# NVIDIA/OpenSeq2Seq

Hardware: AMD Instinct MI355X
Metric: audio-frames/sec/node Jasper10x5 bf16 (train step, objects = input feature frames) (higher is better)
Workload: dtype bf16; 1 GPU; Jasper 10x5 DR (jasper10x5_LibriSpeech_nvgrad_masks) full train step: log-mel front end from int16 PCM resident in HBM+fwd+bwd+NovoGrad/LARC/Backoff, B=32/GPU, durations U[2,16.7]s padded to the batch max, F=64, V=29; global_batch=32, parallelism=dp1, skipped_steps=0

## Files before the change

### openseq2seq_amd/csrc/conv1d_wgrad.hip

```cpp
#include <stdlib.h>

#include <cstdlib>
#include "os2s_common.hpp"
#include "os2s_split_reduce.hpp"
#include <mutex>

namespace os2s {

struct WgradArgs {
  const bf16_t* x;
  const bf16_t* dy;
  float* dw;
  const int32_t* in_len;
  int B, Tin, Tout, Cin, Cout, K, stride, dil, padL;
  int NCO, NCI, NTP, NSPLIT, steps_per_split, use_atomic;
  float* part;
  int xrows, xrows_pad;
  int xbuf_bytes, steptab_bytes;
  long long x_ld;
  int accumulate;
  float* ws_slabs;
  int* ws_cnt;
  int ws_nslabs, ncu, force_split;
  int xcd_order;
  int NG;
  const bf16_t* gx[8];
  const bf16_t* gdy[8];
  float* gdw[8];
  unsigned long long* dbg;
  int dbg_mode;
};

__device__ __forceinline__ int wgrad_xcd_rank(int b, int n) {
  const int q = n >> 3, r = n & 7, x = b & 7;
  return (x < r ? x * (q + 1) : r * (q + 1) + (x - r) * q) + (b >> 3);
}

__device__ __forceinline__ void dma16w(const void* gsrc, char* lds_wave_base) {
  __builtin_amdgcn_global_load_lds(
      (const __attribute__((address_space(1))) void*)gsrc,
      (__attribute__((address_space(3))) void*)lds_wave_base, 16, 0, 0);
}

__device__ __forceinline__ bf16x4 lds_tr(const char* p) {
  return __builtin_amdgcn_ds_read_tr16_b64_v4bf16(
      (__attribute__((address_space(3))) bf16x4*)p);
}

template <int TAPS, int COT>
__device__ __forceinline__ void wgrad_lockstep_unit(const WgradArgs& p, const int unit, const int tp, char* smem) {
  constexpr int BT = 64;
  constexpr int NW = COT / 32, NTHR = NW * 64, NSUB = COT / 128;
  const int tid = threadIdx.x, lane = tid & 63;
  const int wid = __builtin_amdgcn_readfirstlane(tid >> 6);
  const int wm = wid >> 1, wn = wid & 1;
  const int ysub = wm >> 1, wmi = wm & 1;
  const int split = unit / (p.NCO * p.NCI);
  const int rem = unit - split * (p.NCO * p.NCI);
  const int co0 = (rem / p.NCI) * COT, ci0 = (rem % p.NCI) * 128;
  const int k0 = tp * TAPS;
  const int ntaps = min(TAPS, p.K - k0);

  const int ybuf_bytes = NSUB * BT * 256;
  const int xbuf_bytes = p.xrows_pad * 256;
  char* const ybuf0 = smem;
  char* const xbuf0 = smem + 2 * ybuf_bytes;
  const char* const zero = reinterpret_cast<const char*>(g_zero_page);

  const int tchunks = (p.Tout + BT - 1) / BT;
  auto nlive = [&](int b) -> int {
    if (!p.in_len) return tchunks;
    const int l = min(max(p.in_len[b], 0), p.Tin);
    if (l <= 0) return 0;
    return min(tchunks, (l + p.padL + BT * p.stride - 1) / (BT * p.stride));
  };
  int total_live = 0;
  for (int b = 0; b < p.B; ++b) total_live += nlive(b);
  const int sps = (total_live + p.NSPLIT - 1) / p.NSPLIT;
  const int s_begin = split * sps;
  const int s_end = min(total_live, s_begin + sps);
  const int nsteps = max(0, s_end - s_begin);
  int cur_b = 0, cur_c = 0;
  {
    int acc_steps = 0;
    while (cur_b < p.B && acc_steps + nlive(cur_b) <= s_begin) { acc_steps += nlive(cur_b); ++cur_b; }
    cur_c = s_begin - acc_steps;
  }

  auto stage = [&](int step, int buf) {
    const int b = min(cur_b, p.B - 1);
    const int t0 = cur_c * BT;
    ++cur_c;
    if (cur_c >= nlive(b)) {
      cur_c = 0;
      ++cur_b;
      while (cur_b < p.B && nlive(cur_b) == 0) ++cur_b;
    }
    int len_b = p.Tin;
    if (p.in_len) {
      int l = p.in_len[b];
      len_b = l < 0 ? 0 : (l < p.Tin ? l : p.Tin);
    }
    char* yd = ybuf0 + buf * ybuf_bytes;
    const bf16_t* dyb = p.dy + (long long)b * p.Tout * p.Cout;
#pragma unroll
    for (int it = 0; it < (NSUB * 16) / NW; ++it) {
      const int base = (it * NW + wid) * 64;
// ... 142 lines not shown
  const bf16_t* x;
  const bf16_t* dy;
  float* dw;
  long long x_ld;
  int Cin, Cout, NCI, unit_begin;
};
struct WgradGroupTable {
  int ngroups, total_units;
  WgradGroup g[kMaxWgradGroups];
};

__global__ __launch_bounds__(256, 2) void conv1d_wgrad_grouped_kernel(WgradArgs p, WgradGroupTable gt) {
  extern __shared__ __attribute__((aligned(16))) char smem[];
  const int bid = blockIdx.x;
  if (bid >= gt.total_units) return;
  int gi = 0;
#pragma unroll
  for (int i = 1; i < kMaxWgradGroups; ++i)
    if (i < gt.ngroups && bid >= gt.g[i].unit_begin) gi = i;
  WgradGroup g = gt.g[0];
#pragma unroll
  for (int i = 1; i < kMaxWgradGroups; ++i)
    if (i == gi) g = gt.g[i];
  p.x = g.x; p.dy = g.dy; p.dw = g.dw; p.x_ld = g.x_ld;
  p.Cin = g.Cin; p.Cout = g.Cout;
  p.NCO = (g.Cout + 127) / 128; p.NCI = g.NCI;
  wgrad_lockstep_unit<1, 128>(p, bid - g.unit_begin, 0, smem);
}

template <int OFF>
__device__ __forceinline__ bf16x4 lds_tr_asm(unsigned addr) {
  bf16x4 v;
  asm volatile("ds_read_b64_tr_b16 %0, %1 offset:%2" : "=v"(v) : "v"(addr), "n"(OFF) : "memory");
  return v;
}
template <int KK>
__device__ __forceinline__ bf16x8 lds_frag(unsigned addr) {
  const bf16x4 lo = lds_tr_asm<KK * 4096>(addr);
  const bf16x4 hi = lds_tr_asm<KK * 4096 + 1024>(addr);
  return __builtin_shufflevector(lo, hi, 0, 1, 2, 3, 4, 5, 6, 7);
}

__device__ __forceinline__ void wpp_barrier() {
  __builtin_amdgcn_sched_barrier(0);
  __builtin_amdgcn_s_barrier();
  __builtin_amdgcn_sched_barrier(0);
}

constexpr int kWppTaps = 4;
struct WppStaged {
  unsigned ylo, yhi, ynr, xlo, xhi, xnr;
  int xro;
};

template <bool DBG>
__global__ __launch_bounds__(512, 2) void conv1d_wgrad_pp_kernel(WgradArgs p) {
  constexpr int BT = 64, COT = 128, CIT = 128;
  constexpr int YBUF = BT * 256;
  extern __shared__ __attribute__((aligned(16))) char smem[];
  const int tid = threadIdx.x, lane = tid & 63;
  const int wid = __builtin_amdgcn_readfirstlane(tid >> 6);
  const int grp = wid >> 2, wq = wid & 3;
  const int wm = wq >> 1, wn = wq & 1;

  const int tchunks = (p.Tout + BT - 1) / BT;
  int nl = 0, len_l = 0;
  if (lane < p.B) {
    len_l = p.Tin;
    if (p.in_len) {
      const int l = p.in_len[lane];
      len_l = l < 0 ? 0 : (l < p.Tin ? l : p.Tin);
    }
    nl = len_l > 0 ? (len_l + p.padL + BT - 1) / BT : 0;
    nl = nl < tchunks ? nl : tchunks;
  }
  int scan = nl;
#pragma unroll
  for (int o = 1; o < 64; o <<= 1) {
    const int t = __shfl_up(scan, o, 64);
    if (lane >= o) scan += t;
  }
  const int total_live = __builtin_amdgcn_readlane(scan, 63);

  const int U = p.NG * p.NCO * p.NCI * p.NTP, G = p.ncu;
  const int q = U / G, r = U - q * G;
  int f = 1;
  {
    int fmax = total_live / 8;
    fmax = fmax > 16 ? 16 : fmax;
    if (p.force_split > 0 && p.ws_slabs) {
      f = p.force_split < fmax ? p.force_split : (fmax > 1 ? fmax : 1);
      while (f > 1 && r * f > p.ws_nslabs) --f;
      if (r == 0) f = 1;
    } else if (r > 0 && p.ws_slabs) {
      f = split_factor(r, G, 1.1f * total_live, fmax, p.ws_nslabs);
    }
  }
  const int nfull = f > 1 ? U - r : U;
  const int nwork = nfull + (f > 1 ? r * f : 0);
  if ((int)blockIdx.x >= nwork) return;
  const int bid = p.xcd_order ? wgrad_xcd_rank(blockIdx.x, nwork) : (int)blockIdx.x;
  int rank = bid, piece = 0, npiece = 1;
  if (bid >= nfull) {
    const int i = bid - nfull;
    rank = nfull + i / f;
    piece = i - (i / f) * f;
    npiece = f;
  }
  const int tp = rank % p.NTP;
  int rem = rank / p.NTP;
  if (p.NG > 1) {
    const int per = p.NCO * p.NCI;
    const int g = __builtin_amdgcn_readfirstlane(rem / per);
    rem -= g * per;
    const bf16_t* sx = p.gx[0]; const bf16_t* sdy = p.gdy[0]; float* sdw = p.gdw[0];
#pragma unroll
    for (int i = 1; i < 8; ++i)
      if (i == g) { sx = p.gx[i]; sdy = p.gdy[i]; sdw = p.gdw[i]; }
    p.x = sx; p.dy = sdy; p.dw = sdw;
  }
  const int co0 = (rem / p.NCI) * COT, ci0 = (rem % p.NCI) * CIT;
  const int k0 = tp * kWppTaps;
  const int sps = (total_live + npiece - 1) / npiece;
  const int s_begin = __builtin_amdgcn_readfirstlane(min(piece * sps, total_live));
  const int s_end = __builtin_amdgcn_readfirstlane(min(total_live, s_begin + sps));
  const int nsteps = s_end - s_begin;

  const int xbuf_bytes = p.xbuf_bytes;
  char* const ybuf0 = smem;
  char* const xbuf0 = smem + 2 * YBUF;
  int* const steptab = reinterpret_cast<int*>(xbuf0 + 3 * xbuf_bytes);

  {
    const int excl = scan - nl;
    for (int c = 0; c < tchunks; ++c) {
      const int idx = excl + c - s_begin;
      if (lane < p.B && c < nl && idx >= 0 && idx < nsteps && wid == 0)
        steptab[idx] = lane | (c << 8) | (len_l << 16);
    }
  }

  int yv[2];
#pragma unroll
  for (int it = 0; it < 2; ++it) {
    const int qq = (it * 8 + wid) * 64 + lane;
    const int row = qq >> 4, ps = qq & 15;
    const int u = (ps >> 1) ^ ((row & 3) << 1);
    const int ch = co0 + ((u << 1) | (ps & 1)) * 8;
    yv[it] = ch < p.Cout ? (row * p.Cout + ch) * 2 : (int)0x80000000;
  }
  int xv[3];
#pragma unroll
  for (int n = 0; n < 3; ++n) {
    const int qq = (n * 8 + wid) * 64 + lane;
    const int row = qq >> 4, ps = qq & 15;
    const int u = (ps >> 1) ^ ((row & 3) << 1);
    const int ch = ci0 + ((u << 1) | (ps & 1)) * 8;
    xv[n] = (ch < p.Cin && row < p.xrows) ? (row * (int)p.x_ld + ch) * 2 : (int)0x80000000;
  }
  const bool x3 = 16 + wid < ((p.xrows * 16 + 63) >> 6);
  const unsigned long long dy_base = (unsigned long long)p.dy, x_base = (unsigned long long)p.x;
  const int ycol_bytes = __builtin_amdgcn_readfirstlane(p.Cout * 2);
  const int xcol_bytes = __builtin_amdgcn_readfirstlane((int)p.x_ld * 2);
  const unsigned long long xsample_bytes = (unsigned long long)p.Tin * (unsigned long long)p.x_ld * 2ull;
  auto prep = [&](int ent) __attribute__((always_inline)) -> WppStaged {
    const int b = ent & 0xff, t0 = ((ent >> 8) & 0xff) * BT, len_b = (int)((unsigned)ent >> 16);
    WppStaged st;
    const unsigned long long yb = dy_base + (unsigned long long)(unsigned)(b * p.Tout + t0) * (unsigned)ycol_bytes;
    st.ylo = (unsigned)yb; st.yhi = (unsigned)(yb >> 32);
    st.ynr = (unsigned)((p.Tout - t0) * ycol_bytes);
    const unsigned long long xb = x_base + (unsigned long long)(unsigned)b * xsample_bytes;
    st.xlo = (unsigned)xb; st.xhi = (unsigned)(xb >> 32);
    st.xnr = (unsigned)(len_b * xcol_bytes);
    st.xro = (t0 + k0 * p.dil - p.padL) * xcol_bytes;
#if defined(__HIP_DEVICE_COMPILE__)
    asm volatile("" : "+s"(st.ylo), "+s"(st.yhi), "+s"(st.ynr), "+s"(st.xlo), "+s"(st.xhi), "+s"(st.xnr), "+s"(st.xro));
#endif
    return st;
  };
  auto issue = [&](const WppStaged& st, int ybuf_idx, int xbuf_idx) __attribute__((always_inline)) {
    const __amdgpu_buffer_rsrc_t yrs = __builtin_amdgcn_make_buffer_rsrc(
        (void*)(((unsigned long long)st.yhi << 32) | st.ylo), 0, (int)st.ynr, 0x00020000);
    const __amdgpu_buffer_rsrc_t xrs = __builtin_amdgcn_make_buffer_rsrc(
        (void*)(((unsigned long long)st.xhi << 32) | st.xlo), 0, (int)st.xnr, 0x00020000);
    char* const yd = ybuf0 + ybuf_idx * YBUF;
    if (!(DBG && (p.dbg_mode & 1)))
#pragma unroll
    for (int it = 0; it < 2; ++it)
      __builtin_amdgcn_raw_ptr_buffer_load_lds(
          yrs, (__attribute__((address_space(3))) void*)(yd + (it * 8 + wid) * 1024), 16, yv[it], 0, 0, 0);
    char* const xd = xbuf0 + xbuf_idx * xbuf_bytes;
    if (!(DBG && (p.dbg_mode & 2))) {
#pragma unroll
      for (int n = 0; n < 2; ++n)
        __builtin_amdgcn_raw_ptr_buffer_load_lds(
            xrs, (__attribute__((address_space(3))) void*)(xd + (n * 8 + wid) * 1024), 16,
            xv[n] + st.xro, 0, 0, 0);
      if (x3)
        __builtin_amdgcn_raw_ptr_buffer_load_lds(
            xrs, (__attribute__((address_space(3))) void*)(xd + (16 + wid) * 1024), 16, xv[2] + st.xro, 0, 0, 0);
    }
  };
  auto stage = [&](int ent, int ybuf_idx, int xbuf_idx) __attribute__((always_inline)) {
    issue(prep(ent), ybuf_idx, xbuf_idx);
  };

  const bool live0 = k0 + 2 * grp < p.K, live1 = k0 + 2 * grp + 1 < p.K;
  f32x16 acc[2][2][2];
#pragma unroll
  for (int e = 0; e < 2; ++e)
#pragma unroll
    for (int i = 0; i < 2; ++i)
#pragma unroll
      for (int j = 0; j < 2; ++j)
#pragma unroll
        for (int v = 0; v < 16; ++v) acc[e][i][j][v] = 0.f;

  const int lhi = lane >> 5;
  if (nsteps > 0) {
    const int g16 = (lane >> 4) & 1;
    const int i16 = lane & 15;
    const int rsub = i16 >> 2;
    const int csub = (i16 & 3) * 8;
    int ya[2], xa[2][2];
#pragma unroll
    for (int i = 0; i < 2; ++i) {
      const int u = 4 * wm + 2 * i + g16;
      ya[i] = (lhi * 8 + rsub) * 256 + ((u ^ ((rsub & 3) << 1)) << 5) + csub;
    }
#pragma unroll
    for (int e = 0; e < 2; ++e) {
      const int r0 = lhi * 8 + rsub + (2 * grp + e) * p.dil;
#pragma unroll
      for (int j = 0; j < 2; ++j) {
        const int u = 4 * wn + 2 * j + g16;
        xa[e][j] = r0 * 256 + ((u ^ ((r0 & 3) << 1)) << 5) + csub;
      }
    }
    __syncthreads();
    stage(__builtin_amdgcn_readfirstlane(steptab[0]), 0, 0);
    if (nsteps > 1) stage(__builtin_amdgcn_readfirstlane(steptab[1]), 1, 1);
    asm volatile("s_waitcnt vmcnt(0)" ::: "memory");
    __syncthreads();
    if (grp) wpp_barrier();

    const unsigned lds0 = (unsigned)(size_t)(__attribute__((address_space(3))) void*)smem;
    unsigned long long* const tl = reinterpret_cast<unsigned long long*>(xbuf0 + 3 * xbuf_bytes + p.steptab_bytes);
    const unsigned tab0 = lds0 + 2 * YBUF + 3 * xbuf_bytes;
    const bool rec = DBG && p.dbg && bid < 4 && lane == 0 && (wid & 3) == 0;
    auto stamp = [&](int s, int i) {
      if (DBG && rec && s < 48) tl[(grp * 48 + s) * 10 + i] = __builtin_readcyclecounter();
    };
    int xi = 0;
    for (int s = 0; s < nsteps; ++s) {
      const unsigned ys = lds0 + (s & 1) * YBUF;
      const unsigned xs = lds0 + 2 * YBUF + xi * xbuf_bytes;
      bf16x8 xf[2][4], yf[2][4];
      int ent_v;
      asm volatile("ds_read_b32 %0, %1" : "=v"(ent_v) : "v"(tab0 + (s + 2 < nsteps ? s + 2 : s) * 4) : "memory");
      if (live0) {
#pragma unroll
        for (int i = 0; i < 2; ++i) {
          yf[i][0] = lds_frag<0>(ys + ya[i]); yf[i][1] = lds_frag<1>(ys + ya[i]);
          yf[i][2] = lds_frag<2>(ys + ya[i]); yf[i][3] = lds_frag<3>(ys + ya[i]);
        }
#pragma unroll
        for (int j = 0; j < 2; ++j) {
          xf[j][0] = lds_frag<0>(xs + xa[0][j]); xf[j][1] = lds_frag<1>(xs + xa[0][j]);
          xf[j][2] = lds_frag<2>(xs + xa[0][j]); xf[j][3] = lds_frag<3>(xs + xa[0][j]);
        }
      }
      asm volatile("s_waitcnt lgkmcnt(0)" ::: "memory");
      stamp(s, 0);
      wpp_barrier();
      stamp(s, 1);
      WppStaged nxt;
      if (live0) {
#pragma unroll
        for (int kk = 0; kk < 4; ++kk)
#pragma unroll
          for (int i = 0; i < 2; ++i)
#pragma unroll
            for (int j = 0; j < 2; ++j)
              acc[0][i][j] = __builtin_amdgcn_mfma_f32_32x32x16_bf16(yf[i][kk], xf[j][kk], acc[0][i][j], 0, 0, 0);
        nxt = prep(__builtin_amdgcn_readfirstlane(ent_v));
#pragma unroll
        for (int i = 0; i < 16; ++i) {
          __builtin_amdgcn_sched_group_barrier(0x008, 1, 0);
          __builtin_amdgcn_sched_group_barrier(0x004, 3, 0);
          __builtin_amdgcn_sched_group_barrier(0x002, 1, 0);
        }
      } else {
        nxt = prep(__builtin_amdgcn_readfirstlane(ent_v));
      }
      if (DBG) __builtin_amdgcn_sched_barrier(0);
      stamp(s, 2);
      wpp_barrier();
      stamp(s, 3);
      if (live1) {
#pragma unroll
        for (int j = 0; j < 2; ++j) {
          xf[j][0] = lds_frag<0>(xs + xa[1][j]); xf[j][1] = lds_frag<1>(xs + xa[1][j]);
          xf[j][2] = lds_frag<2>(xs + xa[1][j]); xf[j][3] = lds_frag<3>(xs + xa[1][j]);
        }
      }
      asm volatile("s_waitcnt vmcnt(0)" ::: "memory");
      if (DBG) { asm volatile("s_waitcnt lgkmcnt(0)" ::: "memory"); stamp(s, 4); }
      {
        int x2 = xi + 2;
        x2 = x2 >= 3 ? x2 - 3 : x2;
        if (s + 2 < nsteps) issue(nxt, s & 1, x2);
        xi = xi + 1 >= 3 ? 0 : xi + 1;
      }
      stamp(s, 5);
      asm volatile("s_waitcnt lgkmcnt(0)" ::: "memory");
      stamp(s, 6);
      wpp_barrier();
      stamp(s, 7);
      if (live1) {
#pragma unroll
        for (int kk = 0; kk < 4; ++kk)
#pragma unroll
          for (int i = 0; i < 2; ++i)
#pragma unroll
            for (int j = 0; j < 2; ++j)
              acc[1][i][j] = __builtin_amdgcn_mfma_f32_32x32x16_bf16(yf[i][kk], xf[j][kk], acc[1][i][j], 0, 0, 0);
      }
      stamp(s, 8);
      wpp_barrier();
      stamp(s, 9);
    }
    if (!grp) wpp_barrier();
    if (DBG && p.dbg && bid < 4) {
      __syncthreads();
      for (int i = tid; i < 2 * 48 * 10; i += 512) p.dbg[bid * 2 * 48 * 10 + i] = tl[i];
    }
  }
  __syncthreads();

  if (npiece > 1) {
    const int sidx = rank - nfull;
    auto at = [&](int v) -> f32x16& { return acc[v >> 2][(v >> 1) & 1][v & 1]; };
    if (!split_publish_and_reduce(at, p.ws_slabs + (size_t)sidx * f * kSplitSlabFloats,
                                  p.ws_cnt + sidx, piece, f, smem, tid))
      return;
  }

  const int l31 = lane & 31;
  const bool inside = __builtin_amdgcn_readfirstlane((co0 + 128 <= p.Cout && ci0 + 128 <= p.Cin) ? 1 : 0);
#pragma unroll
  for (int e = 0; e < 2; ++e) {
    const int tap = k0 + 2 * grp + e;
    if (tap < p.K) {
      float* const dwk = p.dw + (long long)tap * p.Cout * p.Cin;
      if (inside) {
        float* const base = dwk + (long long)(co0 + wm * 64 + 4 * lhi) * p.Cin + ci0 + wn * 64 + l31;
        float old[2][2][16];
        if (p.accumulate) {
#pragma unroll
          for (int i = 0; i < 2; ++i)
#pragma unroll
            for (int j = 0; j < 2; ++j)
#pragma unroll
              for (int v = 0; v < 16; ++v)
                old[i][j][v] = base[(long long)(i * 32 + (v & 3) + 8 * (v >> 2)) * p.Cin + j * 32];
#pragma unroll
          for (int i = 0; i < 2; ++i)
#pragma unroll
            for (int j = 0; j < 2; ++j)
#pragma unroll
              for (int v = 0; v < 16; ++v) acc[e][i][j][v] += old[i][j][v];
        }
#pragma unroll
        for (int i = 0; i < 2; ++i)
#pragma unroll
          for (int j = 0; j < 2; ++j)
#pragma unroll
            for (int v = 0; v < 16; ++v)
              base[(long long)(i * 32 + (v & 3) + 8 * (v >> 2)) * p.Cin + j * 32] = acc[e][i][j][v];
      } else {
#pragma unroll
        for (int i = 0; i < 2; ++i)
#pragma unroll
          for (int j = 0; j < 2; ++j) {
            const int ci = ci0 + wn * 64 + j * 32 + l31;
#pragma unroll
            for (int v = 0; v < 16; ++v) {
              const int co = co0 + wm * 64 + i * 32 + (v & 3) + 8 * (v >> 2) + 4 * lhi;
              if (co < p.Cout && ci < p.Cin) {
                float* dst = dwk + (long long)co * p.Cin + ci;
                float val = acc[e][i][j][v];
                if (p.accumulate) val += *dst;
                *dst = val;
              }
            }
          }
      }
    }
  }
}

#include "conv1d_wgrad_sw.hpp"

__global__ __launch_bounds__(512, 2) void conv1d_wgrad1x1_pp_kernel(WgradArgs p, WgradGroupTable gt) {
  constexpr int BT = 64;
  constexpr int TILE = BT * 256 * 2;
  constexpr int HALF = TILE / 2;
  extern __shared__ __attribute__((aligned(16))) char smem[];
  const int tid = threadIdx.x, lane = tid & 63;
  const int wid = __builtin_amdgcn_readfirstlane(tid >> 6);
  const int grp = wid >> 2, wn = wid & 3;

  const int tchunks = (p.Tout + BT - 1) / BT;
  int nl = 0, len_l = 0;
  if (lane < p.B) {
    len_l = p.Tout;
    if (p.in_len) {
      const int l = p.in_len[lane];
      len_l = l < 0 ? 0 : (l < p.Tout ? l : p.Tout);
    }
    nl = (len_l + BT - 1) / BT;
    nl = nl < tchunks ? nl : tchunks;
  }
  int scan = nl;
#pragma unroll
  for (int o = 1; o < 64; o <<= 1) {
    const int t = __shfl_up(scan, o, 64);
    if (lane >= o) scan += t;
  }
  const int total_live = __builtin_amdgcn_readlane(scan, 63);

  const int U = p.NCO * p.NCI, G = p.ncu;
  const int q = U / G, r = U - q * G;
  int f = 1;
  {
    int fmax = total_live / 8;
    fmax = fmax > 16 ? 16 : fmax;
    if (p.force_split > 0 && p.ws_slabs) {
      f = p.force_split < fmax ? p.force_split : (fmax > 1 ? fmax : 1);
      while (f > 1 && r * f > p.ws_nslabs) --f;
      if (r == 0) f = 1;
    } else if (r > 0 && p.ws_slabs) {
      f = split_factor(r, G, 1.1f * total_live, fmax, p.ws_nslabs);
    }
  }
  const int nfull = f > 1 ? U - r : U;
  const int nwork = nfull + (f > 1 ? r * f : 0);
  if ((int)blockIdx.x >= nwork) return;
  const int bid = p.xcd_order ? wgrad_xcd_rank(blockIdx.x, nwork) : (int)blockIdx.x;
  int rank = bid, piece = 0, npiece = 1;
  if (bid >= nfull) {
    const int i = bid - nfull;
    rank = nfull + i / f;
    piece = i - (i / f) * f;
    npiece = f;
  }
  int grank = rank;
  if (gt.ngroups > 0) {
    int gi = 0;
#pragma unroll
    for (int i = 1; i < kMaxWgradGroups; ++i)
      if (i < gt.ngroups && rank >= gt.g[i].unit_begin) gi = i;
    WgradGroup g = gt.g[0];
#pragma unroll
    for (int i = 1; i < kMaxWgradGroups; ++i)
      if (i == gi) g = gt.g[i];
    p.x = g.x; p.dy = g.dy; p.dw = g.dw; p.x_ld = g.x_ld;
    p.Cin = g.Cin; p.Cout = g.Cout; p.NCI = g.NCI;
// ... 170 lines not shown

  if (npiece > 1) {
    const int sidx = rank - nfull;
    auto at = [&](int v) -> f32x16& { return acc[v >> 2][(v >> 1) & 1][v & 1]; };
    if (!split_publish_and_reduce(at, p.ws_slabs + (size_t)sidx * f * kSplitSlabFloats,
                                  p.ws_cnt + sidx, piece, f, smem, tid))
      return;
  }

  const int l31 = lane & 31;
  const bool inside = __builtin_amdgcn_readfirstlane((co0 + 256 <= p.Cout && ci0 + 256 <= p.Cin) ? 1 : 0);
#pragma unroll
  for (int e = 0; e < 2; ++e) {
    const int cob = co0 + grp * 128 + e * 64, cib = ci0 + wn * 64;
    if (inside) {
      float* const base = p.dw + (long long)(cob + 4 * lhi) * p.Cin + cib + l31;
      float old[2][2][16];
      if (p.accumulate) {
#pragma unroll
        for (int i = 0; i < 2; ++i)
#pragma unroll
          for (int j = 0; j < 2; ++j)
#pragma unroll
            for (int v = 0; v < 16; ++v)
              old[i][j][v] = base[(long long)(i * 32 + (v & 3) + 8 * (v >> 2)) * p.Cin + j * 32];
#pragma unroll
        for (int i = 0; i < 2; ++i)
#pragma unroll
          for (int j = 0; j < 2; ++j)
#pragma unroll
            for (int v = 0; v < 16; ++v) acc[e][i][j][v] += old[i][j][v];
      }
#pragma unroll
      for (int i = 0; i < 2; ++i)
#pragma unroll
        for (int j = 0; j < 2; ++j)
#pragma unroll
          for (int v = 0; v < 16; ++v)
            base[(long long)(i * 32 + (v & 3) + 8 * (v >> 2)) * p.Cin + j * 32] = acc[e][i][j][v];
    } else {
#pragma unroll
      for (int i = 0; i < 2; ++i)
#pragma unroll
        for (int j = 0; j < 2; ++j) {
          const int ci = cib + j * 32 + l31;
#pragma unroll
          for (int v = 0; v < 16; ++v) {
            const int co = cob + i * 32 + (v & 3) + 8 * (v >> 2) + 4 * lhi;
            if (co < p.Cout && ci < p.Cin) {
              float* dst = p.dw + (long long)co * p.Cin + ci;
              float val = acc[e][i][j][v];
              if (p.accumulate) val += *dst;
              *dst = val;
            }
          }
        }
    }
  }
}

}

static int conv1d_wgrad_impl(os2s_stream_t stream, const uint16_t* x, long long x_row_stride,
                             const uint16_t* dy, float* dw, const int32_t* in_len, int B,
                             int Tin, int Cin, int Cout, int K, int stride, int dil,
                             int padL, int Tout, int accumulate, void* workspace,
                             size_t workspace_bytes);

static int wgrad_pp_min_units() {
  static const int v = [] { const char* e = getenv("OS2S_WGRAD_PP_MIN_UNITS"); return e ? atoi(e) : 8; }();
  return v;
}
static bool wgrad1x1_pp_auto(int B, int T, int Cin, int Cout, bool have_ws) {
  static const int mode = [] { const char* e = getenv("OS2S_WGRAD1X1_PP"); return e ? atoi(e) : -1; }();
  if (mode == 0) return false;
  if (mode == 1) return true;
  const long long rows = (long long)B * T;
  const int units = os2s::ceil_div(Cout, 256) * os2s::ceil_div(Cin, 256);
  return have_ws && rows >= 2048 && units >= 32;
}
static int g_wgrad_variant = -1;
static int g_wgrad_split = -1;
static int g_wgrad_sw_ablate = 0;
static int g_wgrad_xcd = 1;
static unsigned long long* g_wgrad_dbg = nullptr;
static int g_wgrad_dbg_mode = 0;
static os2s::OptionReg r_wg_variant("conv1d_wgrad.variant", [](double v) { g_wgrad_variant = (int)v; });
static os2s::OptionReg r_wg_split("conv1d_wgrad.split", [](double v) { g_wgrad_split = (int)v; });
static os2s::OptionReg r_wg_abl("conv1d_wgrad.sw_ablate", [](double v) { g_wgrad_sw_ablate = (int)v; });
static os2s::OptionReg r_wg_xcd("conv1d_wgrad.xcd_order", [](double v) { g_wgrad_xcd = v != 0 ? 1 : 0; });
static os2s::StampReg r_wg_stamps("conv1d_wgrad", [](void* stamps, int mode) {
  g_wgrad_dbg = (unsigned long long*)stamps;
  g_wgrad_dbg_mode = mode;
});

extern "C" int os2s_conv1d_wgrad_ws(os2s_stream_t stream, const uint16_t* x, long long x_row_stride,
                                    const uint16_t* dy, float* dw, const int32_t* in_len, int B,
                                    int Tin, int Cin, int Cout, int K, int stride, int dil,
                                    int padL, int Tout, int accumulate, void* workspace,
                                    size_t workspace_bytes) {
  return conv1d_wgrad_impl(stream, x, x_row_stride, dy, dw, in_len, B, Tin, Cin, Cout, K, stride,
                           dil, padL, Tout, accumulate, workspace, workspace_bytes);
}

extern "C" int os2s_conv1d_wgrad_ex(os2s_stream_t stream, const uint16_t* x, long long x_row_stride,
                                    const uint16_t* dy, float* dw, const int32_t* in_len, int B,
                                    int Tin, int Cin, int Cout, int K, int stride, int dil,
                                    int padL, int Tout, int accumulate) {
  return conv1d_wgrad_impl(stream, x, x_row_stride, dy, dw, in_len, B, Tin, Cin, Cout, K, stride,
                           dil, padL, Tout, accumulate, nullptr, 0);
}

extern "C" int os2s_conv1d_wgrad(os2s_stream_t stream, const uint16_t* x,
                                 const uint16_t* dy, float* dw,
                                 const int32_t* in_len, int B, int Tin, int Cin,
                                 int Cout, int K, int stride, int dil, int padL,
                                 int Tout, int accumulate) {
  return conv1d_wgrad_impl(stream, x, Cin, dy, dw, in_len, B, Tin, Cin, Cout, K, stride, dil,
                           padL, Tout, accumulate, nullptr, 0);
}

static int conv1d_wgrad_impl_g(os2s_stream_t stream, const uint16_t* x, long long x_row_stride,
                               const uint16_t* dy, float* dw, const int32_t* in_len, int B,
                               int Tin, int Cin, int Cout, int K, int stride, int dil,
                               int padL, int Tout, int accumulate, void* workspace,
                               size_t workspace_bytes, const os2s_cwgrad_group_t* groups, int ngroups);

static int conv1d_wgrad_impl(os2s_stream_t stream, const uint16_t* x, long long x_row_stride,
                             const uint16_t* dy, float* dw, const int32_t* in_len, int B,
                             int Tin, int Cin, int Cout, int K, int stride, int dil,
                             int padL, int Tout, int accumulate, void* workspace,
                             size_t workspace_bytes) {
  return conv1d_wgrad_impl_g(stream, x, x_row_stride, dy, dw, in_len, B, Tin, Cin, Cout, K, stride, dil, padL, Tout,
                             accumulate, workspace, workspace_bytes, nullptr, 1);
}

extern "C" int os2s_conv1d_wgrad_grouped_ws(os2s_stream_t stream, const os2s_cwgrad_group_t* groups, int ngroups,
                                            const int32_t* in_len, int B, int Tin, int Cin, int Cout, int K,
                                            int stride, int dil, int padL, int Tout, int accumulate,
                                            void* workspace, size_t workspace_bytes) {
  OS2S_REQUIRE(groups && ngroups >= 1 && ngroups <= 8);
  for (int i = 0; i < ngroups; ++i) OS2S_REQUIRE(groups[i].x && groups[i].dy && groups[i].dw);
  for (int i = 1; i < ngroups; ++i) OS2S_REQUIRE(groups[i].x_row_stride == groups[0].x_row_stride);
  int rc = OS2S_ERR_UNSUPPORTED;
  if (ngroups > 1)
    rc = conv1d_wgrad_impl_g(stream, groups[0].x, groups[0].x_row_stride, groups[0].dy, groups[0].dw, in_len, B, Tin,
                             Cin, Cout, K, stride, dil, padL, Tout, accumulate, workspace, workspace_bytes, groups,
                             ngroups);
  if (rc != OS2S_ERR_UNSUPPORTED) return rc;
  for (int i = 0; i < ngroups; ++i) {
    rc = conv1d_wgrad_impl(stream, groups[i].x, groups[i].x_row_stride, groups[i].dy, groups[i].dw, in_len, B, Tin,
                           Cin, Cout, K, stride, dil, padL, Tout, accumulate, workspace, workspace_bytes);
    if (rc != OS2S_OK) return rc;
  }
  return OS2S_OK;
}

static int conv1d_wgrad_impl_g(os2s_stream_t stream, const uint16_t* x, long long x_row_stride,
                               const uint16_t* dy, float* dw, const int32_t* in_len, int B,
                               int Tin, int Cin, int Cout, int K, int stride, int dil,
                               int padL, int Tout, int accumulate, void* workspace,
                               size_t workspace_bytes, const os2s_cwgrad_group_t* groups, int ngroups) {
  using namespace os2s;
  OS2S_REQUIRE(x_row_stride >= Cin && x_row_stride % 8 == 0);
  OS2S_REQUIRE(x && dy && dw);
  OS2S_REQUIRE(B >= 0 && Tin >= 1 && Tout >= 1 && Cin >= 8 && Cout >= 8 && K >= 1);
  OS2S_REQUIRE(Cin % 8 == 0 && Cout % 8 == 0 && stride >= 1 && dil >= 1);
  if (B == 0) return OS2S_OK;
  WgradArgs a;
  a.x = x; a.dy = dy; a.dw = dw; a.in_len = in_len;
  a.B = B; a.Tin = Tin; a.Tout = Tout; a.Cin = Cin; a.Cout = Cout; a.K = K;
  a.stride = stride; a.dil = dil; a.padL = padL; a.x_ld = x_row_stride;
  a.accumulate = accumulate ? 1 : 0;
  a.part = nullptr; a.ws_slabs = nullptr; a.ws_cnt = nullptr; a.ws_nslabs = 0; a.ncu = 256; a.force_split = g_wgrad_split;
  a.dbg = g_wgrad_dbg; a.dbg_mode = g_wgrad_dbg_mode; a.xcd_order = g_wgrad_xcd; a.NG = 1;
  for (int i = 0; i < 8; ++i) { a.gx[i] = nullptr; a.gdy[i] = nullptr; a.gdw[i] = nullptr; }
  if (groups) {
    a.NG = ngroups;
    for (int i = 0; i < ngroups; ++i) { a.gx[i] = groups[i].x; a.gdy[i] = groups[i].dy; a.gdw[i] = groups[i].dw; }
  }

  const bool pp_shape = stride == 1 && K >= 2 && B <= 64 && Cout >= 128 && Cin >= 64 &&
                        Tin < 65536 && Tout <= 255 * 64 && 63 + 3 * dil + 1 <= 96 &&
                        (long long)Tin * x_row_stride * 2 < (1ll << 30) &&
                        (long long)Tin * x_row_stride * 2 < (1ll << 31) &&
                        (long long)Tout * Cout * 2 < (1ll << 31);
  const int pp_units = ceil_div(Cout, 128) * ceil_div(Cin, 128) * ceil_div(K, kWppTaps);
  const bool sw_shape = pp_shape && 63 + 3 * dil + 1 <= kSwXInstr * 16 &&
                        Cout % 128 == 0 && Cin % 128 == 0;
  if (sw_shape && g_wgrad_variant == 3 && !groups) {
    a.NCO = ceil_div(Cout, 128);
    a.NCI = ceil_div(Cin, 128);
    a.NTP = ceil_div(K, kWppTaps);
    a.NSPLIT = 1; a.steps_per_split = 0; a.use_atomic = 0;
    a.xrows = 63 + (kWppTaps - 1) * dil + 1;
    a.xrows_pad = ceil_div(a.xrows, 4) * 4;
    a.xbuf_bytes = kSwXBuf;
    a.steptab_bytes = ceil_div(B * ceil_div(Tout, 64) * 4, 16) * 16;
    const size_t smem = (size_t)kSwRing * (kSwYBuf + kSwXBuf) + a.steptab_bytes;
    if (smem <= 160 * 1024) {
      static std::once_flag once_sw;
      static hipError_t attr_rc = hipSuccess;
      static int ncu = 256;
      std::call_once(once_sw, [] {
        attr_rc = hipFuncSetAttribute((const void*)conv1d_wgrad_sw_kernel<0>,
                                      hipFuncAttributeMaxDynamicSharedMemorySize, 160 * 1024);
#ifdef OS2S_SW_ABLATE
        for (const void* k : {(const void*)conv1d_wgrad_sw_kernel<1>, (const void*)conv1d_wgrad_sw_kernel<2>,
                              (const void*)conv1d_wgrad_sw_kernel<4>, (const void*)conv1d_wgrad_sw_kernel<8>,
                              (const void*)conv1d_wgrad_sw_kernel<3>, (const void*)conv1d_wgrad_sw_kernel<5>})
          if (attr_rc == hipSuccess) attr_rc = hipFuncSetAttribute(k, hipFuncAttributeMaxDynamicSharedMemorySize, 160 * 1024);
#endif
        int dev = 0, n = 0;
        if (hipGetDevice(&dev) == hipSuccess &&
            hipDeviceGetAttribute(&n, hipDeviceAttributeMultiprocessorCount, dev) == hipSuccess && n > 0)
          ncu = n;
      });
      if (attr_rc != hipSuccess) return OS2S_ERR_LAUNCH;
      a.ncu = ncu;
      const size_t slab_bytes = (size_t)kSplitSlabFloats * 4;
      if (workspace && workspace_bytes >= kSplitTicketBytes + 2 * slab_bytes) {
        a.ws_cnt = reinterpret_cast<int*>(workspace);
        a.ws_slabs = reinterpret_cast<float*>(reinterpret_cast<char*>(workspace) + kSplitTicketBytes);
        size_t n = (workspace_bytes - kSplitTicketBytes) / slab_bytes;
        const size_t cap = (size_t)3 * ncu;
        a.ws_nslabs = (int)(n < cap ? n : cap);
      }
      const int U = a.NCO * a.NCI * a.NTP;
      const int r = U % ncu;
      const int pieces = a.ws_nslabs < 16 * r ? a.ws_nslabs : 16 * r;
#ifdef OS2S_SW_ABLATE
      switch (g_wgrad_sw_ablate) {
        case 1: OS2S_LAUNCH(conv1d_wgrad_sw_kernel<1>, dim3(U + pieces), dim3(256), smem, (hipStream_t)stream, a); return OS2S_OK;
        case 2: OS2S_LAUNCH(conv1d_wgrad_sw_kernel<2>, dim3(U + pieces), dim3(256), smem, (hipStream_t)stream, a); return OS2S_OK;
        case 3: OS2S_LAUNCH(conv1d_wgrad_sw_kernel<3>, dim3(U + pieces), dim3(256), smem, (hipStream_t)stream, a); return OS2S_OK;
        case 4: OS2S_LAUNCH(conv1d_wgrad_sw_kernel<4>, dim3(U + pieces), dim3(256), smem, (hipStream_t)stream, a); return OS2S_OK;
        case 5: OS2S_LAUNCH(conv1d_wgrad_sw_kernel<5>, dim3(U + pieces), dim3(256), smem, (hipStream_t)stream, a); return OS2S_OK;
        case 8: OS2S_LAUNCH(conv1d_wgrad_sw_kernel<8>, dim3(U + pieces), dim3(256), smem, (hipStream_t)stream, a); return OS2S_OK;
        default: break;
      }
#endif
      OS2S_LAUNCH(conv1d_wgrad_sw_kernel<0>, dim3(U + pieces), dim3(256), smem, (hipStream_t)stream, a);
      return OS2S_OK;
    }
  }

  if (pp_shape && g_wgrad_variant != 0 && (groups || g_wgrad_variant == 1 || pp_units >= wgrad_pp_min_units())) {
    a.NCO = ceil_div(Cout, 128);
    a.NCI = ceil_div(Cin, 128);
    a.NTP = ceil_div(K, kWppTaps);
    a.NSPLIT = 1; a.steps_per_split = 0; a.use_atomic = 0;
    a.xrows = 63 + (kWppTaps - 1) * dil + 1;
    a.xrows_pad = ceil_div(a.xrows, 4) * 4;
    a.xbuf_bytes = 24 * 1024;
    a.steptab_bytes = ceil_div(B * ceil_div(Tout, 64) * 4, 16) * 16;
    const size_t smem = (size_t)2 * 64 * 256 + (size_t)3 * a.xbuf_bytes + a.steptab_bytes + (a.dbg ? 2 * 48 * 10 * 8 : 0);
    if (smem <= 160 * 1024) {
      static std::once_flag once;
      static hipError_t attr_rc = hipSuccess;
      static int ncu = 256;
      std::call_once(once, [] {
        attr_rc = hipFuncSetAttribute((const void*)conv1d_wgrad_pp_kernel<false>,
                                      hipFuncAttributeMaxDynamicSharedMemorySize, 160 * 1024);
        if (attr_rc == hipSuccess)
          attr_rc = hipFuncSetAttribute((const void*)conv1d_wgrad_pp_kernel<true>,
                                        hipFuncAttributeMaxDynamicSharedMemorySize, 160 * 1024);
        int dev = 0, n = 0;
        if (hipGetDevice(&dev) == hipSuccess &&
            hipDeviceGetAttribute(&n, hipDeviceAttributeMultiprocessorCount, dev) == hipSuccess && n > 0)
          ncu = n;
      });
      if (attr_rc != hipSuccess) return OS2S_ERR_LAUNCH;
      a.ncu = ncu;
      const size_t slab_bytes = (size_t)kSplitSlabFloats * 4;
      if (workspace && workspace_bytes >= kSplitTicketBytes + 2 * slab_bytes) {
        a.ws_cnt = reinterpret_cast<int*>(workspace);
        a.ws_slabs = reinterpret_cast<float*>(reinterpret_cast<char*>(workspace) + kSplitTicketBytes);
        size_t n = (workspace_bytes - kSplitTicketBytes) / slab_bytes;
        const size_t cap = (size_t)3 * ncu;
        a.ws_nslabs = (int)(n < cap ? n : cap);
      }
      const int U = a.NG * a.NCO * a.NCI * a.NTP;
      const int r = U % ncu;
      int pieces = a.ws_nslabs < 16 * r ? a.ws_nslabs : 16 * r;
      const int grid = U + pieces;
      if (a.dbg) {
        OS2S_LAUNCH(conv1d_wgrad_pp_kernel<true>, dim3(grid), dim3(512), smem, (hipStream_t)stream, a);
      } else {
        OS2S_LAUNCH(conv1d_wgrad_pp_kernel<false>, dim3(grid), dim3(512), smem, (hipStream_t)stream, a);
      }
      return OS2S_OK;
    }
  }

  if (groups) return OS2S_ERR_UNSUPPORTED;

  const bool pp1_shape = K == 1 && stride == 1 && padL == 0 && Tin == Tout && B <= 64 &&
                         Cout >= 128 && Cin >= 128 && x_row_stride * 2 * 64 < (1ll << 30) &&
                         (long long)Cout * 2 * 64 < (1ll << 30);
  if (pp1_shape && g_wgrad_variant != 0 && g_wgrad_variant != 1 &&
      (g_wgrad_variant == 2 || wgrad1x1_pp_auto(B, Tout, Cin, Cout, workspace != nullptr))) {
    a.NCO = ceil_div(Cout, 256);
    a.NCI = ceil_div(Cin, 256);
    a.NTP = 1;
    a.NSPLIT = 1; a.steps_per_split = 0; a.use_atomic = 0;
    a.xrows = 64; a.xrows_pad = 64; a.xbuf_bytes = 0; a.steptab_bytes = 0;
    static std::once_flag once1;
    static hipError_t attr_rc1 = hipSuccess;
    static int ncu1 = 256;
    std::call_once(once1, [] {
      attr_rc1 = hipFuncSetAttribute((const void*)conv1d_wgrad1x1_pp_kernel,
                                     hipFuncAttributeMaxDynamicSharedMemorySize, 160 * 1024);
      int dev = 0, n = 0;
      if (hipGetDevice(&dev) == hipSuccess &&
          hipDeviceGetAttribute(&n, hipDeviceAttributeMultiprocessorCount, dev) == hipSuccess && n > 0)
        ncu1 = n;
    });
    if (attr_rc1 != hipSuccess) return OS2S_ERR_LAUNCH;
    a.ncu = ncu1;
    const size_t slab_bytes = (size_t)kSplitSlabFloats * 4;
    if (workspace && workspace_bytes >= kSplitTicketBytes + 2 * slab_bytes) {
      a.ws_cnt = reinterpret_cast<int*>(workspace);
      a.ws_slabs = reinterpret_cast<float*>(reinterpret_cast<char*>(workspace) + kSplitTicketBytes);
      size_t n = (workspace_bytes - kSplitTicketBytes) / slab_bytes;
      const size_t cap = (size_t)3 * ncu1;
      a.ws_nslabs = (int)(n < cap ? n : cap);
    }
    const int U = a.NCO * a.NCI;
    const int r = U % ncu1;
    const int pieces = a.ws_nslabs < 16 * r ? a.ws_nslabs : 16 * r;
    WgradGroupTable none;
    none.ngroups = 0; none.total_units = 0;
    OS2S_LAUNCH(conv1d_wgrad1x1_pp_kernel, dim3(U + pieces), dim3(512), (size_t)160 * 1024,
                (hipStream_t)stream, a, none);
    return OS2S_OK;
  }

  const int TAPS = K == 1 ? 1 : 2;
  const bool wide = (Cout % 256 == 0) && (K >= 8) && (Cout >= 512);
  const int COT = wide ? 256 : 128;
  a.NCO = ceil_div(Cout, COT);
  a.NCI = ceil_div(Cin, 128);
  a.NTP = ceil_div(K, TAPS);
  const int base_blocks = a.NCO * a.NCI * a.NTP;
  const int total_steps = B * ceil_div(Tout, 64);
  int nsplit = 1;
  if (accumulate) {
    const int target = wide ? 256 : 512;
    nsplit = ceil_div(target, base_blocks);
    const int max_split = total_steps / 8 > 0 ? total_steps / 8 : 1;
    if (nsplit > max_split) nsplit = max_split;
    if (nsplit < 1) nsplit = 1;
    if (os2s_deterministic()) nsplit = 1;
  }
  const long long dw_elems = (long long)K * Cout * Cin;
  if (workspace) {
    const long long part_room = workspace_bytes > kSplitTicketBytes
                                    ? (long long)((workspace_bytes - kSplitTicketBytes) / ((size_t)dw_elems * 4)) : 0;
    if (nsplit > part_room) nsplit = (int)part_room;
    if (nsplit < 1) nsplit = 1;
  }
  a.steps_per_split = ceil_div(total_steps, nsplit);
  a.NSPLIT = ceil_div(total_steps, a.steps_per_split);
  if (workspace && a.NSPLIT > 1)
    a.part = reinterpret_cast<float*>(reinterpret_cast<char*>(workspace) + kSplitTicketBytes);
// ... 216 lines not shown
```

Before: 942,800 frames/sec.

## Pack tail-tap wgrad tiles across two Cin blocks and spread full tiles across XCDs

When K leaves a single leftover tap per tap-pass (K % kWppTaps == 1), the wgrad pp kernel now pairs two adjacent Cin tiles into one work unit for that last tap. Each wave group handles a different Cin block, so half-idle tail units are no longer launched. The x staging buffer grows to 32KB with a fourth load slot to hold both Cin slices. A new xcd_order mode 2, now the default, applies the XCD-aware rank remap only to the full tiles and leaves split pieces in launch order. The cost is more LDS per block, which can lower occupancy, and extra index logic.

```diff
diff --git a/openseq2seq_amd/csrc/conv1d_wgrad.hip b/openseq2seq_amd/csrc/conv1d_wgrad.hip
--- a/openseq2seq_amd/csrc/conv1d_wgrad.hip
+++ b/openseq2seq_amd/csrc/conv1d_wgrad.hip
@@ -23,6 +23,7 @@
   int* ws_cnt;
   int ws_nslabs, ncu, force_split;
   int xcd_order;
+  int per_co, pack_tail;
   int NG;
   const bf16_t* gx[8];
   const bf16_t* gdy[8];
@@ -331,7 +332,7 @@
   }
   const int total_live = __builtin_amdgcn_readlane(scan, 63);
 
-  const int U = p.NG * p.NCO * p.NCI * p.NTP, G = p.ncu;
+  const int U = p.NG * p.NCO * p.per_co, G = p.ncu;
   const int q = U / G, r = U - q * G;
   int f = 1;
   {
@@ -348,7 +349,9 @@
   const int nfull = f > 1 ? U - r : U;
   const int nwork = nfull + (f > 1 ? r * f : 0);
   if ((int)blockIdx.x >= nwork) return;
-  const int bid = p.xcd_order ? wgrad_xcd_rank(blockIdx.x, nwork) : (int)blockIdx.x;
+  const bool spread = p.xcd_order == 2 && f > 1 && nfull > 0;
+  const int bid = spread ? ((int)blockIdx.x < nfull ? wgrad_xcd_rank(blockIdx.x, nfull) : (int)blockIdx.x)
+                         : (p.xcd_order ? wgrad_xcd_rank(blockIdx.x, nwork) : (int)blockIdx.x);
   int rank = bid, piece = 0, npiece = 1;
   if (bid >= nfull) {
     const int i = bid - nfull;
@@ -356,8 +359,23 @@
     piece = i - (i / f) * f;
     npiece = f;
   }
-  const int tp = rank % p.NTP;
-  int rem = rank / p.NTP;
+  int tp, rem;
+  bool tail = false;
+  if (p.pack_tail) {
+    const int nq = p.NTP - 1, blk = 2 * nq + 1;
+    const int row = rank / p.per_co, rr = rank - row * p.per_co;
+    const int m = rr / blk, w = rr - m * blk;
+    int ci = 2 * m;
+    tp = w;
+    if (2 * m + 1 < p.NCI) {
+      tail = w == 2 * nq;
+      if (w >= nq) { tp = w - nq; ci += tail ? 0 : 1; }
+    }
+    rem = row * p.NCI + ci;
+  } else {
+    tp = rank % p.NTP;
+    rem = rank / p.NTP;
+  }
   if (p.NG > 1) {
     const int per = p.NCO * p.NCI;
     const int g = __builtin_amdgcn_readfirstlane(rem / per);
@@ -369,7 +387,9 @@
     p.x = sx; p.dy = sdy; p.dw = sdw;
   }
   const int co0 = (rem / p.NCI) * COT, ci0 = (rem % p.NCI) * CIT;
-  const int k0 = tp * kWppTaps;
+  const int k0 = tail ? p.K - 1 : tp * kWppTaps;
+  const int tap0 = tail ? p.K - 1 : k0 + 2 * grp;
+  const int ci0w = tail ? ci0 + grp * CIT : ci0;
   const int sps = (total_live + npiece - 1) / npiece;
   const int s_begin = __builtin_amdgcn_readfirstlane(min(piece * sps, total_live));
   const int s_end = __builtin_amdgcn_readfirstlane(min(total_live, s_begin + sps));
@@ -398,16 +418,19 @@
     const int ch = co0 + ((u << 1) | (ps & 1)) * 8;
     yv[it] = ch < p.Cout ? (row * p.Cout + ch) * 2 : (int)0x80000000;
   }
-  int xv[3];
-#pragma unroll
-  for (int n = 0; n < 3; ++n) {
+  int xv[4];
+#pragma unroll
+  for (int n = 0; n < 4; ++n) {
     const int qq = (n * 8 + wid) * 64 + lane;
-    const int row = qq >> 4, ps = qq & 15;
+    const int lrow = qq >> 4, ps = qq & 15;
+    const int row = tail ? lrow & 63 : lrow;
     const int u = (ps >> 1) ^ ((row & 3) << 1);
-    const int ch = ci0 + ((u << 1) | (ps & 1)) * 8;
-    xv[n] = (ch < p.Cin && row < p.xrows) ? (row * (int)p.x_ld + ch) * 2 : (int)0x80000000;
-  }
-  const bool x3 = 16 + wid < ((p.xrows * 16 + 63) >> 6);
+    const int ch = ci0 + (tail ? (lrow >> 6) * CIT : 0) + ((u << 1) | (ps & 1)) * 8;
+    xv[n] = (ch < p.Cin && (tail || row < p.xrows)) ? (row * (int)p.x_ld + ch) * 2 : (int)0x80000000;
+  }
+  const int nxi = tail ? 32 : (p.xrows * 16 + 63) >> 6;
+  const bool x3 = 16 + wid < nxi;
+  const bool x4 = 24 + wid < nxi;
   const unsigned long long dy_base = (unsigned long long)p.dy, x_base = (unsigned long long)p.x;
   const int ycol_bytes = __builtin_amdgcn_readfirstlane(p.Cout * 2);
   const int xcol_bytes = __builtin_amdgcn_readfirstlane((int)p.x_ld * 2);
@@ -448,13 +471,16 @@
       if (x3)
         __builtin_amdgcn_raw_ptr_buffer_load_lds(
             xrs, (__attribute__((address_space(3))) void*)(xd + (16 + wid) * 1024), 16, xv[2] + st.xro, 0, 0, 0);
+      if (x4)
+        __builtin_amdgcn_raw_ptr_buffer_load_lds(
+            xrs, (__attribute__((address_space(3))) void*)(xd + (24 + wid) * 1024), 16, xv[3] + st.xro, 0, 0, 0);
     }
   };
   auto stage = [&](int ent, int ybuf_idx, int xbuf_idx) __attribute__((always_inline)) {
     issue(prep(ent), ybuf_idx, xbuf_idx);
   };
 
-  const bool live0 = k0 + 2 * grp < p.K, live1 = k0 + 2 * grp + 1 < p.K;
+  const bool live0 = tap0 < p.K, live1 = tap0 + 1 < p.K;
   f32x16 acc[2][2][2];
 #pragma unroll
   for (int e = 0; e < 2; ++e)
@@ -479,11 +505,11 @@
     }
 #pragma unroll
     for (int e = 0; e < 2; ++e) {
-      const int r0 = lhi * 8 + rsub + (2 * grp + e) * p.dil;
+      const int r0 = lhi * 8 + rsub + (tail ? 0 : (2 * grp + e) * p.dil);
 #pragma unroll
       for (int j = 0; j < 2; ++j) {
         const int u = 4 * wn + 2 * j + g16;
-        xa[e][j] = r0 * 256 + ((u ^ ((r0 & 3) << 1)) << 5) + csub;
+        xa[e][j] = r0 * 256 + ((u ^ ((r0 & 3) << 1)) << 5) + csub + (tail ? grp * (BT * 256) : 0);
       }
     }
     __syncthreads();
@@ -596,14 +622,14 @@
   }
 
   const int l31 = lane & 31;
-  const bool inside = __builtin_amdgcn_readfirstlane((co0 + 128 <= p.Cout && ci0 + 128 <= p.Cin) ? 1 : 0);
+  const bool inside = __builtin_amdgcn_readfirstlane((co0 + 128 <= p.Cout && ci0w + 128 <= p.Cin) ? 1 : 0);
 #pragma unroll
   for (int e = 0; e < 2; ++e) {
-    const int tap = k0 + 2 * grp + e;
+    const int tap = tap0 + e;
     if (tap < p.K) {
       float* const dwk = p.dw + (long long)tap * p.Cout * p.Cin;
       if (inside) {
-        float* const base = dwk + (long long)(co0 + wm * 64 + 4 * lhi) * p.Cin + ci0 + wn * 64 + l31;
+        float* const base = dwk + (long long)(co0 + wm * 64 + 4 * lhi) * p.Cin + ci0w + wn * 64 + l31;
         float old[2][2][16];
         if (p.accumulate) {
 #pragma unroll
@@ -632,7 +658,7 @@
         for (int i = 0; i < 2; ++i)
 #pragma unroll
           for (int j = 0; j < 2; ++j) {
-            const int ci = ci0 + wn * 64 + j * 32 + l31;
+            const int ci = ci0w + wn * 64 + j * 32 + l31;
 #pragma unroll
             for (int v = 0; v < 16; ++v) {
               const int co = co0 + wm * 64 + i * 32 + (v & 3) + 8 * (v >> 2) + 4 * lhi;
@@ -969,13 +995,15 @@
 static int g_wgrad_variant = -1;
 static int g_wgrad_split = -1;
 static int g_wgrad_sw_ablate = 0;
-static int g_wgrad_xcd = 1;
+static int g_wgrad_xcd = 2;
+static int g_wgrad_pack_tail = 1;
 static unsigned long long* g_wgrad_dbg = nullptr;
 static int g_wgrad_dbg_mode = 0;
 static os2s::OptionReg r_wg_variant("conv1d_wgrad.variant", [](double v) { g_wgrad_variant = (int)v; });
 static os2s::OptionReg r_wg_split("conv1d_wgrad.split", [](double v) { g_wgrad_split = (int)v; });
 static os2s::OptionReg r_wg_abl("conv1d_wgrad.sw_ablate", [](double v) { g_wgrad_sw_ablate = (int)v; });
-static os2s::OptionReg r_wg_xcd("conv1d_wgrad.xcd_order", [](double v) { g_wgrad_xcd = v != 0 ? 1 : 0; });
+static os2s::OptionReg r_wg_xcd("conv1d_wgrad.xcd_order", [](double v) { g_wgrad_xcd = v >= 2 ? 2 : (v != 0 ? 1 : 0); });
+static os2s::OptionReg r_wg_pack("conv1d_wgrad.pack_tail", [](double v) { g_wgrad_pack_tail = v != 0 ? 1 : 0; });
 static os2s::StampReg r_wg_stamps("conv1d_wgrad", [](void* stamps, int mode) {
   g_wgrad_dbg = (unsigned long long*)stamps;
   g_wgrad_dbg_mode = mode;
@@ -1061,6 +1089,7 @@
   a.accumulate = accumulate ? 1 : 0;
   a.part = nullptr; a.ws_slabs = nullptr; a.ws_cnt = nullptr; a.ws_nslabs = 0; a.ncu = 256; a.force_split = g_wgrad_split;
   a.dbg = g_wgrad_dbg; a.dbg_mode = g_wgrad_dbg_mode; a.xcd_order = g_wgrad_xcd; a.NG = 1;
+  a.per_co = 0; a.pack_tail = 0;
   for (int i = 0; i < 8; ++i) { a.gx[i] = nullptr; a.gdy[i] = nullptr; a.gdw[i] = nullptr; }
   if (groups) {
     a.NG = ngroups;
@@ -1139,9 +1168,17 @@
     a.NSPLIT = 1; a.steps_per_split = 0; a.use_atomic = 0;
     a.xrows = 63 + (kWppTaps - 1) * dil + 1;
     a.xrows_pad = ceil_div(a.xrows, 4) * 4;
-    a.xbuf_bytes = 24 * 1024;
+    a.pack_tail = (g_wgrad_pack_tail && K % kWppTaps == 1 && a.NCI >= 2) ? 1 : 0;
+    a.per_co = a.pack_tail ? a.NCI * (a.NTP - 1) + ceil_div(a.NCI, 2) : a.NCI * a.NTP;
     a.steptab_bytes = ceil_div(B * ceil_div(Tout, 64) * 4, 16) * 16;
-    const size_t smem = (size_t)2 * 64 * 256 + (size_t)3 * a.xbuf_bytes + a.steptab_bytes + (a.dbg ? 2 * 48 * 10 * 8 : 0);
+    a.xbuf_bytes = 32 * 1024;
+    size_t smem = (size_t)2 * 64 * 256 + (size_t)3 * a.xbuf_bytes + a.steptab_bytes + (a.dbg ? 2 * 48 * 10 * 8 : 0);
+    if (!a.pack_tail || smem > 160 * 1024) {
+      a.pack_tail = 0;
+      a.per_co = a.NCI * a.NTP;
+      a.xbuf_bytes = 24 * 1024;
+      smem -= 3 * 8 * 1024;
+    }
     if (smem <= 160 * 1024) {
       static std::once_flag once;
       static hipError_t attr_rc = hipSuccess;
@@ -1167,7 +1204,7 @@
         const size_t cap = (size_t)3 * ncu;
         a.ws_nslabs = (int)(n < cap ? n : cap);
       }
-      const int U = a.NG * a.NCO * a.NCI * a.NTP;
+      const int U = a.NG * a.NCO * a.per_co;
       const int r = U % ncu;
       int pieces = a.ws_nslabs < 16 * r ? a.ws_nslabs : 16 * r;
       const int grid = U + pieces;
```

New measurement: 946,600 frames/sec, median of 6. No clear change (+0.4%).
